# taipingeric/yolo-v4-tf.keras

Measured on AMD Instinct MI355X. Metric: images/sec end-to-end predict() at 608x608 batch 32; conv MFMA %peak, higher is better.
Workload: dtype bf16

## Files before the change

### yolo-v4-tf.keras_amd/csrc/conv_igemm.hip

```cpp
#include "conv_chain.h"
#include "conv_tiles.h"

namespace y4 {

int conv_launch_f32(int tile, const ConvK& k, hipStream_t s);
int conv_launch_bf16(int tile, const ConvK& k, hipStream_t s);
int conv_launch_f16(int tile, const ConvK& k, hipStream_t s);
int conv_launch_bf16_fused(int tile, const ConvK& k, hipStream_t s);
int conv_launch_f16_fused(int tile, const ConvK& k, hipStream_t s);

template <class F, class... A>
static int launch_16bit(int dtype, const char* who, F* bf16, F* f16, const A&... a) {
    if (dtype == Y4_BF16) return bf16(a...);
    if (dtype == Y4_F16) return f16(a...);
    set_error("conv2d: %s 16-bit only", who);
    return Y4_EINVAL;
}
int conv_p8_launch_bf16(int bm, int nst, const ConvK& k, hipStream_t s);
int conv_p8_launch_f16(int bm, int nst, const ConvK& k, hipStream_t s);
int conv_halo_launch_bf16(int bm, int bn, const ConvK& k, hipStream_t s);
int conv_halo_launch_f16(int bm, int bn, const ConvK& k, hipStream_t s);
int conv_halo2_launch_bf16(int tile, const ConvK& k, hipStream_t s);
int conv_halo2_launch_f16(int tile, const ConvK& k, hipStream_t s);
int conv_p8_launch(int dtype, int bm, int nst, const ConvK& k, hipStream_t s) {
    return launch_16bit(dtype, "the phased kernel is", conv_p8_launch_bf16, conv_p8_launch_f16, bm, nst, k, s);
}
int conv_halo_launch(int dtype, int bm, int bn, const ConvK& k, hipStream_t s) {
    return launch_16bit(dtype, "halo tiles are", conv_halo_launch_bf16, conv_halo_launch_f16, bm, bn, k, s);
}
int conv_halo2_launch(int dtype, int tile, const ConvK& k, hipStream_t s) {
    return launch_16bit(dtype, "halo2 tiles are", conv_halo2_launch_bf16, conv_halo2_launch_f16, tile, k, s);
}

int conv_tile_count() { return kNumTiles; }

bool weight_touch_enabled() {
    static const bool on = [] { const char* e = getenv("Y4_NO_WEIGHT_TOUCH"); return !(e && e[0] == '1'); }();
    return on;
}

static bool tile_ok(const TileCfg& tc, int dtype, int cin, int cout_pad) {
    const int bk = tc.bkb / elem_size(dtype);
    return cin % bk == 0 && cout_pad % tc.bn == 0;
}

static void set_bands(ConvK& k, const HaloPlan& hp, int n) {
    k.h_rows = hp.rows; k.h_bands = hp.bands; k.h_pitch = hp.pitch;
    k.h_div_pitch = fastdiv_make((uint32_t)hp.pitch); k.h_div_bands = fastdiv_make((uint32_t)hp.bands);
    k.grid_m = n * hp.bands;
}

int conv_pick_tile(int dtype, int M, int cin, int cout) {
    const int es = elem_size(dtype);
    const bool k128 = cin % (128 / es) == 0;
    if (cout <= 32) return k128 ? 5 : 6;
    if (cout <= 64) return k128 ? 3 : 4;
    return k128 ? 8 : 9;
}

int conv2d_launch(const y4_conv_desc* d, const char* zero_page, hipStream_t stream, const ConvChainDesc* chain,
                  const ConvPairDesc* pair, const ConvObjDesc* obj) {
    Y4_REQUIRE(d && d->in && d->wt && d->out && d->scale && d->shift, Y4_EINVAL, "conv2d: null pointer");
    Y4_REQUIRE(d->dtype >= Y4_F32 && d->dtype <= Y4_F16, Y4_EINVAL, "conv2d: bad dtype %d", d->dtype);
    Y4_REQUIRE(d->ksize == 1 || d->ksize == 3, Y4_EINVAL, "conv2d: ksize %d (only 1 or 3)", d->ksize);
    Y4_REQUIRE(d->stride == 1 || (d->stride == 2 && d->ksize == 3), Y4_EINVAL, "conv2d: stride %d", d->stride);
    Y4_REQUIRE(d->stride == 1 || (d->h % 2 == 0 && d->w % 2 == 0), Y4_EINVAL, "conv2d: stride 2 needs even h,w");
    Y4_REQUIRE(d->n > 0 && d->h > 0 && d->w > 0 && d->cin > 0 && d->cout > 0, Y4_EINVAL, "conv2d: empty shape");
    const int es = elem_size(d->dtype);
    const int epc = 16 / es;
    Y4_REQUIRE(d->cin % (64 / es) == 0, Y4_EINVAL, "conv2d: cin %d must be a multiple of %d for dtype %d",
               d->cin, 64 / es, d->dtype);
    Y4_REQUIRE(d->cin % k_chunk_channels(d->cin, d->ksize) == 0, Y4_EINVAL,
               "conv2d: cin %d is not a whole number of %d-channel K chunks (the canonical K order of a 3x3 conv, common.h)", d->cin,
               k_chunk_channels(d->cin, d->ksize));
    Y4_REQUIRE(d->in_cstride % epc == 0 && d->in_coff % epc == 0, Y4_EINVAL, "conv2d: input view not 16-byte aligned");
    const int oepc = d->out_f32 ? 4 : epc;
    Y4_REQUIRE(d->out_cstride % oepc == 0 && d->out_coff % oepc == 0, Y4_EINVAL,
               "conv2d: output view not 16-byte aligned");
    Y4_REQUIRE(!d->res || (d->res_cstride % epc == 0 && d->res_coff % epc == 0), Y4_EINVAL,
               "conv2d: residual view not 16-byte aligned");
    ConvK k{};
    k.in = (const char*)d->in; k.wt = (const char*)d->wt; k.scale = d->scale; k.shift = d->shift;
    k.res = (const char*)d->res; k.out = (char*)d->out; k.zero = zero_page;
    k.N = d->n; k.H = d->h; k.W = d->w; k.Cin = d->cin;
    k.Ho = d->h / d->stride; k.Wo = d->w / d->stride;
    k.cout_store = (int)round_up(d->cout, 8);
    Y4_REQUIRE((int64_t)d->n * k.Ho * k.Wo < (1ll << 31), Y4_EINVAL, "conv2d: too many output pixels");
    k.M = d->n * k.Ho * k.Wo;
    k.K = d->ksize * d->ksize * d->cin;
    const int64_t in_bytes = (int64_t)d->n * d->h * d->w * d->in_cstride * es;
    const int64_t wt_bytes = (int64_t)round_up(d->cout, COUT_PAD) * k.K * es;
    const int64_t tap_span = d->ksize == 3 ? ((int64_t)3 * d->w + 3) * d->in_cstride * es + (int64_t)d->cin * es : 0;
    Y4_REQUIRE(in_bytes + tap_span < (1ll << 31) && wt_bytes < (1ll << 31), Y4_EINVAL,
               "conv2d: input (%lld B + %lld B of tap reach) or weights (%lld B) exceed the 2 GiB buffer-descriptor range", (long long)in_bytes,
               (long long)tap_span, (long long)wt_bytes);
    k.in_bytes = (unsigned)in_bytes; k.wt_bytes = (unsigned)wt_bytes;
    {
        const int64_t ob = (int64_t)k.M * d->out_cstride * es, ob2 = d->out2 ? (int64_t)k.M * d->out2_cstride * es : 0,
                      rb = d->res ? (int64_t)k.M * d->res_cstride * es : 0;
        k.fast_epi = !d->upsample && !d->out_f32 && ob < (1ll << 31) && ob2 < (1ll << 31) && rb < (1ll << 31);
        if (k.fast_epi) { k.out_bytes = (unsigned)ob; k.out2_bytes = (unsigned)ob2; k.res_bytes = (unsigned)rb; }
    }
    k.div_howo = fastdiv_make((uint32_t)(k.Ho * k.Wo)); k.div_wo = fastdiv_make((uint32_t)k.Wo);
    k.in_cstride = d->in_cstride; k.in_coff = d->in_coff;
    k.out_cstride = d->out_cstride; k.out_coff = d->out_coff;
    k.res_cstride = d->res_cstride; k.res_coff = d->res_coff;
    k.ksize = d->ksize; k.stride = d->stride; k.pad = d->ksize == 3 ? 1 : 0;
    k.act = d->act; k.upsample = d->upsample; k.out_f32 = d->out_f32;
    if (obj) {
        Y4_REQUIRE(obj->obj && !d->upsample && ((pair && pair->out_f32) || (!pair && d->out_f32)), Y4_EINVAL,
                   "conv2d: an objectness side array needs a float32 head");
        k.obj = obj->obj; k.obj_nf = obj->nf; k.obj_cpi = obj->cells_per_img; k.obj_base = obj->cell_base;
    }
    const int cout_pad = (int)round_up(d->cout, COUT_PAD);
    if (pair) {
        Y4_REQUIRE(!chain && d->dtype != Y4_F32 && (d->cout == 128 || d->cout == 256) && pair->cout >= 1 && pair->cout <= d->cout && !d->upsample &&
                       !d->out_f32 && (!d->out2 || (d->split == 64 && d->cout == 128)) && pair->w && pair->scale && pair->shift && pair->fin &&
                       pair->fin_cstride % (pair->out_f32 ? 4 : epc) == 0 && pair->fin_coff % (pair->out_f32 ? 4 : epc) == 0,
                   Y4_EINVAL, "conv2d: bad LDS-pair description");
        k.pair = pair->out_f32 ? 3 : 1; k.tail_act = pair->act; k.store_x = pair->store_x;
        k.tail[0].w = (const char*)pair->w; k.tail[0].scale = pair->scale; k.tail[0].shift = pair->shift; k.tail[0].cout = (int)round_up(pair->cout, 8);
// ... 211 lines not shown
```

### yolo-v4-tf.keras_amd/csrc/conv_igemm_kernel.h

```cpp
#pragma once
#include "conv_chain.h"
#include "conv_tiles.h"

namespace y4 {

#ifdef Y4_TRACE
__device__ unsigned long long y4_trace_buf[4 * 8 * 8];
__device__ unsigned long long y4_trace_life[8 * 8];
#define TR_LIFE(P, INSN)                                                                                    \
    do {                                                                                                    \
        __builtin_amdgcn_sched_barrier(0);                                                                  \
        if (tr_life_on) asm volatile(INSN " %0" : "=s"(tr_life[P]));                                        \
        __builtin_amdgcn_sched_barrier(0);                                                                  \
    } while (0)
#define TR_KT0 10
#define TR_WG 8
#define TR_POINT(P)                                                                                         \
    do {                                                                                                    \
        __builtin_amdgcn_sched_barrier(0);                                                                  \
        if (tr_on && kt >= TR_KT0 && kt < TR_KT0 + 4) asm volatile("s_memtime %0" : "=s"(tr_t[P]));         \
        __builtin_amdgcn_sched_barrier(0);                                                                  \
    } while (0)
#else
#define TR_POINT(P)
#define TR_LIFE(P, INSN)
#endif

template <int DT, int BM, int BN, int WM, int WN, int BKB, int NST, int CHAIN = 0, bool PAIR = false>
__global__ __launch_bounds__(64 * WM * WN, CHAIN ? 2 : 1) void conv_igemm_kernel(const ConvK p) {
    constexpr int NT = 64 * WM * WN;
    constexpr int ES = (DT == Y4_F32) ? 4 : 2;
    constexpr int BK = BKB / ES;
    constexpr int CPR = BKB / 16;
    constexpr int EPC = 16 / ES;
    constexpr int RPI = NT / CPR;
    constexpr int A_IT = (BM + RPI - 1) / RPI;
    constexpr bool A_PART = BM % RPI != 0;
    constexpr int B_IT = BN >= RPI ? BN / RPI : 1;
    constexpr bool B_PART = BN < RPI;
    constexpr int WPX = BM / WM, WCH = BN / WN;
    constexpr int MREP = WPX / 16, NREP = WCH / 16;
    constexpr int CPL = 4 * NREP;
    constexpr bool PHASED = (NST == 12);
    constexpr bool M32 = (NST == 32);
    constexpr int SN = (PHASED || M32) ? 2 : NST;
    constexpr bool PREFRAG = true;
    constexpr int STAGE = (BM + BN) * BKB;
    constexpr int KSTEPS = BKB / 64;
    static_assert(BM % 16 == 0 && (BN % RPI == 0 || (RPI % BN == 0 && (BN * CPR) % 64 == 0)), "tile rows vs rows-per-iteration");
    constexpr int LDS_MAIN = SN * STAGE + (CHAIN ? ChainShape<CHAIN ? CHAIN : 1>::LDS_BYTES : 0);
    static_assert(MREP >= 1 && NREP >= 1, "wave tile");
    constexpr int LPT = A_IT + B_IT;
    static_assert(SN >= 2 && SN <= 7 && (SN == 2 || !B_PART), "deep pipelines need uniform weight loads per wave");
    static_assert((SN - 2) * LPT <= 63, "vmcnt field");
    static_assert(!PHASED || (NT == 512 && KSTEPS == 2), "phased schedule: 8 waves, 128-byte K rows");
    static_assert(!M32 || (DT != Y4_F32 && BKB == 128 && WPX % 32 == 0 && WCH % 32 == 0 && CHAIN == 0 && !PAIR && !B_PART),
                  "32x32x16 tiles: 16-bit, 128-byte K rows, wave tile in 32x32 blocks, plain launches");

    extern __shared__ __attribute__((aligned(16))) char smem[];

    asm volatile("" ::"s"(p.H), "s"(p.W), "s"(p.Cin), "s"(p.Ho), "s"(p.Wo), "s"(p.M), "s"(p.K), "s"(p.in_cstride), "s"(p.in_coff), "s"(p.ksize),
                 "s"(p.stride), "s"(p.pad), "s"(p.grid_m), "s"(p.grid_n), "s"(p.in_bytes), "s"(p.wt_bytes), "s"(p.ksplit), "s"(p.touch));

    const int nwg = p.grid_m * p.grid_n;
    int t, ks = 0;
    {
        const int b = blockIdx.x, qq = nwg >> 3, rr = nwg & 7, xcd = b & 7;
        int idx = b >> 3;
        if constexpr (CHAIN == 0 && !PAIR && NST != 12 && NST != 32) {
            if (p.ksplit > 1) {
                ks = idx % p.ksplit;
                idx /= p.ksplit;
                if (idx >= qq + (xcd < rr ? 1 : 0)) return;
            }
        }
        t = (xcd < rr ? xcd * (qq + 1) : rr * (qq + 1) + (xcd - rr) * qq) + idx;
    }
    const int tile_m = (int)fastdiv((uint32_t)t, p.div_gridn), tile_n = t - tile_m * p.grid_n;
    const int m0 = tile_m * BM, n0 = tile_n * BN;

    const int tid = threadIdx.x, lane = tid & 63, wave = tid >> 6;
    const int wm = wave / WN, wn = wave - wm * WN;
#ifdef Y4_TRACE
#ifndef Y4_TRACE_PAIR
#define Y4_TRACE_PAIR 0
#endif
    const bool tr_life_on = blockIdx.x == TR_WG && BM == Y4_TRACE_BM && BN == 256 && NST == Y4_TRACE_NST && CHAIN == 0 && PAIR == (Y4_TRACE_PAIR != 0);
    unsigned long long tr_life[8] = {0, 0, 0, 0, 0, 0, 0, 0};
#endif
    TR_LIFE(0, "s_memtime");
    TR_LIFE(5, "s_memrealtime");
    ChainPrefetch<CHAIN != 0 ? MREP : 1> chain_pf;
    if constexpr (CHAIN != 0) {
        chain_stage_weights<CHAIN, WM * WN>(p, smem + SN * STAGE, __builtin_amdgcn_readfirstlane(wave), lane);
        chain_prefetch<DT, MREP, CHAIN>(p, chain_pf, m0 + wm * WPX + (lane & 15), p.M, lane);
    }

    const int q = tid % CPR, r0 = tid / CPR;
    auto tswz = [](int row) { return M32 ? (swz<CPR>(row) ^ ((row >> 4) & 1)) : swz<CPR>(row); };
    int a_off[A_IT], a_mask[A_IT];
    const int HoWo = p.Ho * p.Wo;
#pragma unroll
    for (int j = 0; j < A_IT; ++j) {
        const int row = r0 + j * RPI;
        const int m = m0 + row;
        const int mm = m < p.M ? m : 0;
        const int n = (int)fastdiv((uint32_t)mm, p.div_howo), rem = mm - n * HoWo;
        const int ho = (int)fastdiv((uint32_t)rem, p.div_wo), wo = rem - ho * p.Wo;
        const int hi0 = ho * p.stride - p.pad, wi0 = wo * p.stride - p.pad;
        a_off[j] = (((n * p.H + hi0 + 1) * p.W + wi0 + 1) * p.in_cstride + p.in_coff + ((q ^ tswz(row)) * EPC)) * ES;
        int mask = 1;
        if (p.ksize == 3) {
            const int cols = ((unsigned)wi0 < (unsigned)p.W ? 1 : 0) | ((unsigned)(wi0 + 1) < (unsigned)p.W ? 2 : 0) | ((unsigned)(wi0 + 2) < (unsigned)p.W ? 4 : 0);
            mask = ((unsigned)hi0 < (unsigned)p.H ? cols : 0) | ((unsigned)(hi0 + 1) < (unsigned)p.H ? cols << 3 : 0) |
                   ((unsigned)(hi0 + 2) < (unsigned)p.H ? cols << 6 : 0);
        }
        a_mask[j] = m < p.M ? mask : 0;
    }
    int b_off[B_IT];
#pragma unroll
    for (int j = 0; j < B_IT; ++j) {
        const int row = B_PART ? (r0 % BN) : (r0 + j * RPI);
        const int wb = row / WCH, pr = row - wb * WCH;
        int ch;
        if constexpr (M32) {
            const int jb = pr >> 5, R = pr & 31, g = R >> 3, hh = (R >> 2) & 1, jj = R & 3;
            ch = chunk_channel_g<2>(n0 + wb * WCH, 2 * jb + (g >> 1), hh) + (g & 1) * 4 + jj;
        } else {
            const int jn = pr >> 4, i = pr & 15, g = i >> 2, r = i & 3;
            ch = chunk_channel(n0 + wb * WCH, jn >> 1, g) + (jn & 1) * 4 + r;
        }
        b_off[j] = (ch * p.K + ((q ^ tswz(row)) * EPC)) * ES;
    }
    const int tap_bias = (p.W + 1) * p.in_cstride * ES;
    const __amdgpu_buffer_rsrc_t rs_in = make_rsrc(p.in - tap_bias, p.in_bytes + (unsigned)tap_bias);
    const __amdgpu_buffer_rsrc_t rs_wt = make_rsrc(p.wt, p.wt_bytes);
    const int wave_lds = __builtin_amdgcn_readfirstlane(wave * 1024);

    const bool a_skip = A_PART && __builtin_amdgcn_readfirstlane(r0 + (A_IT - 1) * RPI >= BM ? 1 : 0) != 0;
    const int chb = k_chunk_channels(p.Cin, p.ksize) * ES;
    int ky = 0, kx = 0, cbase = 0, c_in = 0, ktb = 0;
    int nk = p.K / BK;
    if constexpr (CHAIN == 0 && !PAIR && NST != 12 && NST != 32) {
        if (p.ksplit > 1) {
            const int kt0 = (int)((int64_t)ks * nk / p.ksplit), kt1 = (int)((int64_t)(ks + 1) * nk / p.ksplit);
            const int per = chb / BKB;
            const int idx = kt0 / per, taps = p.ksize * p.ksize;
            const int chunk = idx / taps, tap = idx - chunk * taps;
            ky = tap / p.ksize; kx = tap - ky * p.ksize;
            cbase = chunk * chb;
            c_in = (kt0 - idx * per) * BKB;
            ktb = kt0 * BKB;
            nk = kt1 - kt0;
        }
    }
    constexpr bool TAPVEC = A_IT <= 2 && SN >= 5;
    typedef int i32x16 __attribute__((ext_vector_type(16)));
    const int cs = p.in_cstride * ES;
    const int step_row = (p.W - (p.ksize - 1)) * cs, step_back = -((p.ksize - 1) * p.W + (p.ksize - 1)) * cs;
    int tap = ky * p.ksize + kx;
    int tap_off = (ky * p.W + kx) * cs;
    int a_vo[A_IT];
    i32x16 a_tapv[TAPVEC ? A_IT : 1];
    if constexpr (TAPVEC) {
#pragma unroll
        for (int j = 0; j < A_IT; ++j)
#pragma unroll
            for (int t = 0; t < 9; ++t) a_tapv[j][t] = ((a_mask[j] >> t) & 1) ? a_off[j] : (int)0x80000000;
    }
    auto set_tap = [&]() {
#pragma unroll
        for (int j = 0; j < A_IT; ++j) {
            if constexpr (TAPVEC) a_vo[j] = a_tapv[j][tap];
            else a_vo[j] = ((a_mask[j] >> tap) & 1) ? a_off[j] : (int)0x80000000;
        }
    };
    set_tap();
    int c0b = cbase + c_in + tap_off;
    auto stage = [&](int buf) {
        const int da = buf * STAGE + wave_lds;
        const int db = da + BM * BKB;
#pragma unroll
        for (int j = 0; j < A_IT; ++j)
            if (!A_PART || r0 + j * RPI < BM)
                buffer_load16_lds(rs_in, smem + da + j * (NT * 16), a_vo[j], c0b);
#pragma unroll
        for (int j = 0; j < B_IT; ++j)
            if (!B_PART || tid < BN * CPR)
                buffer_load16_lds(rs_wt, smem + db + j * (NT * 16), b_off[j], ktb);
        ktb += BKB;
        c_in += BKB;
        if (__builtin_expect(c_in >= chb, 1)) {
            c_in = 0;
            ++tap;
            tap_off += cs;
            if (__builtin_expect(++kx >= p.ksize, 0)) {
                kx = 0;
                tap_off += step_row - cs;
                if (++ky >= p.ksize) { ky = 0; tap = 0; tap_off = 0; cbase += chb; }
            }
            set_tap();
        }
        c0b = cbase + c_in + tap_off;
    };

    if (p.touch != 0) {
        weight_touch(rs_wt, smem + LDS_MAIN, n0 * p.K * ES, BN * p.K * ES, wave, NT / 64, lane);
        if constexpr (PAIR)
            weight_touch(make_rsrc(p.tail[0].w, p.tail_w_bytes), smem + LDS_MAIN, 0, (int)p.tail_w_bytes, wave, NT / 64, lane);
    }

    const int frow = lane & 15, fg = lane >> 4;
    int xo[KSTEPS];
#pragma unroll
    for (int kk = 0; kk < KSTEPS; ++kk) xo[kk] = frow * BKB + (((kk * 4 + fg) ^ swz<CPR>(frow)) * 16);
    const char* const lds_x = smem + (wm * WPX) * BKB;
    const char* const lds_w = smem + BM * BKB + (wn * WCH) * BKB;

    f32x4 acc[MREP][NREP];
#pragma unroll
    for (int i = 0; i < MREP; ++i)
#pragma unroll
        for (int j = 0; j < NREP; ++j) acc[i][j] = f32x4{0.f, 0.f, 0.f, 0.f};

    constexpr bool EARLY_TABLES = CHAIN == 0 && !PAIR && !M32 && !PHASED && NREP <= 2;
    float sc_early[NREP * 4], sh_early[NREP * 4];
    if constexpr (EARLY_TABLES) conv_epilogue_tables<NREP>(p, n0 + wn * WCH, fg, sc_early, sh_early);

    TR_LIFE(1, "s_memtime");
    if constexpr (M32) {
        constexpr int MB = WPX / 32, NB = WCH / 32;
        const int frow32 = lane & 31, fh = lane >> 5;
        int xo32[4];
#pragma unroll
        for (int ks = 0; ks < 4; ++ks) xo32[ks] = frow32 * 128 + (((2 * ks + fh) ^ tswz(frow32)) * 16);
        f32x16 acc32[MB][NB];
#pragma unroll
        for (int i = 0; i < MB; ++i)
#pragma unroll
            for (int j = 0; j < NB; ++j)
#pragma unroll
                for (int e = 0; e < 16; ++e) acc32[i][j][e] = 0.f;
        stage(0);
        for (int kt = 0; kt < nk; ++kt) {
            wait_vmcnt_then_barrier<0>();
            if (kt + 1 < nk) stage((kt + 1) & 1);
            unsigned xa[4], wa[4];
#pragma unroll
            for (int ks = 0; ks < 4; ++ks) {
                xa[ks] = (unsigned)(uintptr_t)(smem + (kt & 1) * STAGE + (wm * WPX) * BKB + xo32[ks]);
                wa[ks] = (unsigned)(uintptr_t)(smem + (kt & 1) * STAGE + (wn * WCH) * BKB + xo32[ks]);
            }
            u32x4 xf[4][MB], wf[4][NB];
#pragma unroll
            for (int ks = 0; ks < 4; ++ks) {
#pragma unroll
                for (int i = 0; i < MB; ++i)
                    asm volatile("ds_read_b128 %0, %1 offset:%2" : "=v"(xf[ks][i]) : "v"(xa[ks]), "n"(i * 32 * 128));
#pragma unroll
                for (int j = 0; j < NB; ++j)
                    asm volatile("ds_read_b128 %0, %1 offset:%2" : "=v"(wf[ks][j]) : "v"(wa[ks]), "n"(BM * BKB + j * 32 * 128));
            }
            __builtin_amdgcn_s_setprio(1);
#pragma unroll
            for (int ks = 0; ks < 4; ++ks) {
                constexpr int R = MB + NB;
                if (ks == 0) asm volatile("s_waitcnt lgkmcnt(%2)" : "+v"(xf[0][0]), "+v"(wf[0][0]) : "n"(3 * R > 15 ? 15 : 3 * R));
                if (ks == 1) asm volatile("s_waitcnt lgkmcnt(%2)" : "+v"(xf[1][0]), "+v"(wf[1][0]) : "n"(2 * R > 15 ? 15 : 2 * R));
                if (ks == 2) asm volatile("s_waitcnt lgkmcnt(%2)" : "+v"(xf[2][0]), "+v"(wf[2][0]) : "n"(R > 15 ? 15 : R));
                if (ks == 3) asm volatile("s_waitcnt lgkmcnt(%2)" : "+v"(xf[3][0]), "+v"(wf[3][0]) : "n"(0));
#pragma unroll
                for (int j = 0; j < NB; ++j)
#pragma unroll
                    for (int i = 0; i < MB; ++i) Mma32<DT>::run(acc32[i][j], wf[ks][j], xf[ks][i]);
                __builtin_amdgcn_sched_barrier(0);
            }
            __builtin_amdgcn_s_setprio(0);
        }
        f32x4 accv[MB][NB * 4];
#pragma unroll
        for (int i = 0; i < MB; ++i)
#pragma unroll
            for (int j = 0; j < NB; ++j)
#pragma unroll
                for (int f = 0; f < 4; ++f)
                    accv[i][j * 4 + f] = f32x4{acc32[i][j][4 * f], acc32[i][j][4 * f + 1], acc32[i][j][4 * f + 2], acc32[i][j][4 * f + 3]};
        const bool full32 = (m0 + BM <= p.M) && (n0 + BN <= p.cout_store);
        conv_epilogue<DT, MB, NB * 4, false, 2>(p, accv, m0 + wm * WPX + frow32, p.M, n0 + wn * WCH, fh, full32);
        return;
    } else if constexpr (PHASED) {
        auto phase_barrier = [] {
            asm volatile("s_barrier" ::: "memory");
            __builtin_amdgcn_sched_barrier(0);
        };
        auto wait_loads = [] { asm volatile("s_waitcnt vmcnt(0)" ::: "memory"); };
        const bool grp1 = __builtin_amdgcn_readfirstlane(wave >= 4 ? 1 : 0) != 0;
        stage(0);
        wait_loads();
        phase_barrier();
        if (grp1) {
            if (nk > 1) stage(1);
            phase_barrier();
        }
        for (int kt = 0; kt < nk; ++kt) {
            const char* sx = lds_x + (kt & 1) * STAGE;
            const char* sw = lds_w + (kt & 1) * STAGE;
            u32x4 xf[MREP], wf[NREP];
            if (!grp1 && kt + 1 < nk) stage((kt + 1) & 1);
#pragma unroll
            for (int i = 0; i < MREP; ++i) xf[i] = *(const u32x4*)(sx + i * 16 * BKB + xo[0]);
#pragma unroll
            for (int j = 0; j < NREP; ++j) wf[j] = *(const u32x4*)(sw + j * 16 * BKB + xo[0]);
            phase_barrier();
// ... 22 lines not shown
        }
        if (!grp1) phase_barrier();
    } else {
#pragma unroll
    for (int s = 0; s < SN - 1; ++s)
        if (s < nk) stage(s);
    int cur = 0, nxt = SN - 1;
#ifdef Y4_TRACE
    const bool tr_on = blockIdx.x == TR_WG && BM == Y4_TRACE_BM && BN == 256 && NST == Y4_TRACE_NST && CHAIN == 0 && !PAIR;
    unsigned long long tr_t[8] = {0, 0, 0, 0, 0, 0, 0, 0};
#endif
    for (int kt = 0; kt < nk; ++kt) {
        TR_POINT(0);
#ifdef Y4_TRACE
        if (tr_on && kt >= TR_KT0 && kt < TR_KT0 + 4) asm volatile("s_memrealtime %0" : "=s"(tr_t[7]));
#endif
        const int ahead = nk - 1 - kt;
#ifdef Y4_TRACE
        if (SN == 2 || ahead == 0) {
            asm volatile("s_waitcnt vmcnt(0)" ::: "memory");
            TR_POINT(4);
            asm volatile("s_barrier" ::: "memory");
        } else
#endif
        if (a_skip) wait_vmcnt_then_barrier_k<SN - 2, LPT - 1>(ahead);
        else wait_vmcnt_then_barrier_k<SN - 2, LPT>(ahead);
        TR_POINT(1);
        if (kt == 0) TR_LIFE(2, "s_memtime");
        constexpr bool READS_FIRST = SN >= 5;
        if (!READS_FIRST && kt + SN - 1 < nk) stage(nxt);
        TR_POINT(2);
        const char* sx = lds_x + cur * STAGE;
        const char* sw = lds_w + cur * STAGE;
        const int nxt_now = nxt;
        cur = cur + 1 == SN ? 0 : cur + 1;
        nxt = nxt + 1 == SN ? 0 : nxt + 1;
        if constexpr (PREFRAG) {
            u32x4 xf[KSTEPS][MREP], wf[KSTEPS][NREP];
#pragma unroll
            for (int kk = 0; kk < KSTEPS; ++kk) {
#pragma unroll
                for (int i = 0; i < MREP; ++i) xf[kk][i] = *(const u32x4*)(sx + i * 16 * BKB + xo[kk]);
#pragma unroll
                for (int j = 0; j < NREP; ++j) wf[kk][j] = *(const u32x4*)(sw + j * 16 * BKB + xo[kk]);
            }
            TR_POINT(3);
            if (READS_FIRST && kt + SN - 1 < nk) stage(nxt_now);
            __builtin_amdgcn_s_setprio(1);
#pragma unroll
            for (int kk = 0; kk < KSTEPS; ++kk)
#pragma unroll
                for (int i = 0; i < MREP; ++i)
#pragma unroll
                    for (int j = 0; j < NREP; ++j) Mma<DT>::run(acc[i][j], wf[kk][j], xf[kk][i]);
            __builtin_amdgcn_s_setprio(0);
            TR_POINT(5);
#ifdef Y4_TRACE
            if (tr_on && kt >= TR_KT0 && kt < TR_KT0 + 4) {
                asm volatile("s_waitcnt lgkmcnt(0)" ::: "memory");
                if (lane == 0)
                    for (int q2 = 0; q2 < 8; ++q2) y4_trace_buf[((kt - TR_KT0) * 8 + wave) * 8 + q2] = tr_t[q2];
            }
#endif
        } else
#pragma unroll
        for (int kk = 0; kk < KSTEPS; ++kk) {
            u32x4 xf[MREP], wf[NREP];
#pragma unroll
            for (int i = 0; i < MREP; ++i) xf[i] = *(const u32x4*)(sx + i * 16 * BKB + xo[kk]);
#pragma unroll
            for (int j = 0; j < NREP; ++j) wf[j] = *(const u32x4*)(sw + j * 16 * BKB + xo[kk]);
#pragma unroll
            for (int i = 0; i < MREP; ++i)
#pragma unroll
                for (int j = 0; j < NREP; ++j) Mma<DT>::run(acc[i][j], wf[j], xf[i]);
        }
    }
    }

    if constexpr (CHAIN != 0) {
        static_assert(WN == 1 && BN == 16 * ChainShape<CHAIN>::HEAD_NREP && DT != Y4_F32,
                      "chain head: one wave column over all its output channels, 16-bit");
        chain_epilogue<DT, MREP, CHAIN>(p, smem + SN * STAGE, acc, chain_pf, m0 + wm * WPX + frow, p.M, lane);
    } else if constexpr (PAIR) {
        static_assert(BKB == 128 && DT != Y4_F32 && SN == 2 && !PHASED && !B_PART, "LDS pair: plain 2-stage, 128-byte rows");
        constexpr int XPANEL = BM * 128, NK2 = BN / 64, XBYTES = NK2 * XPANEL, W2STAGE = BN * 128;
        TR_LIFE(3, "s_memtime");
        __syncthreads();
        char* const xl = smem;
        const int xrow = wm * WPX + frow, mrow = m0 + xrow, chw = wn * WCH;
        int b2_off[B_IT];
#pragma unroll
        for (int j = 0; j < B_IT; ++j) {
            const int row = r0 + j * RPI;
            const int wb = row / WCH, pr = row - wb * WCH;
            const int jn = pr >> 4, i = pr & 15, g = i >> 2, r = i & 3;
            const int ch = chunk_channel(wb * WCH, jn >> 1, g) + (jn & 1) * 4 + r;
            b2_off[j] = (ch * p.tail_k + ((q ^ swz<CPR>(row)) * EPC)) * ES;
        }
        const __amdgpu_buffer_rsrc_t rs_w2 = make_rsrc(p.tail[0].w, p.tail_w_bytes);
        auto stage_w2 = [&](int buf, int kt) {
#pragma unroll
            for (int j = 0; j < B_IT; ++j)
                buffer_load16_lds(rs_w2, smem + XBYTES + buf * W2STAGE + wave_lds + j * (NT * 16), b2_off[j], kt * BKB);
        };
        stage_w2(0, 0);
        conv_epilogue<DT, MREP, NREP, true>(p, acc, mrow, p.M, chw, fg, m0 + BM <= p.M, xl, xrow, XPANEL);
        __syncthreads();
        TR_LIFE(7, "s_memtime");
        f32x4 acc2[MREP][NREP];
#pragma unroll
        for (int i = 0; i < MREP; ++i)
#pragma unroll
            for (int j = 0; j < NREP; ++j) acc2[i][j] = f32x4{0.f, 0.f, 0.f, 0.f};
        const int nk2 = p.tail_k >> 6;
        for (int kt = 0; kt < nk2; ++kt) {
            wait_vmcnt_then_barrier<0>();
            if (kt + 1 < nk2) stage_w2((kt + 1) & 1, kt + 1);
            const char* sx = xl + (p.tail_panel0 + kt) * XPANEL + (wm * WPX) * BKB;
            const char* sw = smem + XBYTES + (kt & 1) * W2STAGE + (wn * WCH) * BKB;
            u32x4 xf[KSTEPS][MREP], wf[KSTEPS][NREP];
#pragma unroll
            for (int kk = 0; kk < KSTEPS; ++kk) {
#pragma unroll
                for (int i = 0; i < MREP; ++i) xf[kk][i] = *(const u32x4*)(sx + i * 16 * BKB + xo[kk]);
#pragma unroll
                for (int j = 0; j < NREP; ++j) wf[kk][j] = *(const u32x4*)(sw + j * 16 * BKB + xo[kk]);
            }
#pragma unroll
            for (int kk = 0; kk < KSTEPS; ++kk)
#pragma unroll
                for (int i = 0; i < MREP; ++i)
#pragma unroll
                    for (int j = 0; j < NREP; ++j) Mma<DT>::run(acc2[i][j], wf[kk][j], xf[kk][i]);
        }
#if defined(Y4_TRACE) && Y4_TRACE_PAIR
        TR_LIFE(0, "s_memtime");
#endif
        ConvK p2 = p;
        p2.scale = p.tail[0].scale; p2.shift = p.tail[0].shift; p2.act = p.tail_act; p2.res = nullptr;
        p2.out = p.fin; p2.out_cstride = p.fin_cstride; p2.out_coff = p.fin_coff;
        p2.cout_store = p.tail[0].cout; p2.upsample = 0; p2.out_f32 = p.pair >> 1;
        p2.split = p.tail_split; p2.out2 = p.fin2; p2.out2_cstride = p.fin2_cstride; p2.out2_coff = p.fin2_coff;
        p2.fast_epi = p.fast_tail; p2.out_bytes = p.fin_bytes; p2.out2_bytes = p.fin2_bytes;
        conv_epilogue<DT, MREP, NREP>(p2, acc2, mrow, p.M, chw, fg, (m0 + BM <= p.M) && BN <= p2.cout_store);
#if defined(Y4_TRACE) && Y4_TRACE_PAIR
        TR_LIFE(1, "s_memtime");
#endif
        if (p.store_x) pair_store_tile<DT, MREP, NREP>(p, xl, xrow, XPANEL, mrow, p.M, chw, fg);
        TR_LIFE(4, "s_memtime");
        TR_LIFE(6, "s_memrealtime");
#ifdef Y4_TRACE
        if (tr_life_on) {
            asm volatile("s_waitcnt lgkmcnt(0)" ::: "memory");
            if (lane == 0)
                for (int q2 = 0; q2 < 8; ++q2) y4_trace_life[wave * 8 + q2] = tr_life[q2];
        }
#endif
    } else {
        TR_LIFE(3, "s_memtime");
        if constexpr (NST != 12 && NST != 32) {
            if (p.ksplit > 1) {
                constexpr int FR = MREP * NREP;
                f32x4* const mine = (f32x4*)p.part + ((size_t)ks * nwg + t) * FR * NT + tid;
#pragma unroll
                for (int i = 0; i < MREP; ++i)
#pragma unroll
                    for (int j = 0; j < NREP; ++j) store16_agent(mine + (i * NREP + j) * NT, acc[i][j]);
                asm volatile("s_waitcnt vmcnt(0)" ::: "memory");
                __syncthreads();
                int* const flag = (int*)smem;
                if (tid == 0) {
                    const int old = atomicAdd(p.split_cnt + t, 1);
                    if (old == p.ksplit - 1) p.split_cnt[t] = 0;
                    *flag = old == p.ksplit - 1;
                }
                __syncthreads();
                if (*flag == 0) return;
                const f32x4* src = (const f32x4*)p.part + (size_t)t * FR * NT + tid;
                for (int sp = 0; sp < p.ksplit; ++sp) {
#pragma unroll
                    for (int i = 0; i < MREP; ++i) {
                        f32x4 part[NREP];
#pragma unroll
                        for (int j = 0; j < NREP; ++j) part[j] = load16_agent(src + (i * NREP + j) * NT);
#pragma unroll
                        for (int j = 0; j < NREP; ++j) acc[i][j] = sp == 0 ? part[j] : acc[i][j] + part[j];
                    }
                    src += (size_t)nwg * FR * NT;
                }
            }
        }
        const bool full = (m0 + BM <= p.M) && (n0 + BN <= p.cout_store);
        if constexpr (EARLY_TABLES) conv_epilogue_with<DT, MREP, NREP>(p, acc, sc_early, sh_early, m0 + wm * WPX + frow, p.M, n0 + wn * WCH, fg, full);
        else conv_epilogue<DT, MREP, NREP>(p, acc, m0 + wm * WPX + frow, p.M, n0 + wn * WCH, fg, full);
        TR_LIFE(4, "s_memtime");
        TR_LIFE(6, "s_memrealtime");
#ifdef Y4_TRACE
        if (tr_life_on) {
            asm volatile("s_waitcnt lgkmcnt(0)" ::: "memory");
            if (lane == 0)
                for (int q2 = 0; q2 < 8; ++q2) y4_trace_life[wave * 8 + q2] = tr_life[q2];
        }
#endif
    }
}

template <int DT, int BM, int BN, int WM, int WN, int BKB, int NST, int CHAIN = 0, bool PAIR = false>
static int launch_cfg(const ConvK& k, hipStream_t stream) {
    constexpr int lds_main = (NST == 12 || NST == 32 ? 2 : NST) * (BM + BN) * BKB + (CHAIN ? ChainShape<CHAIN ? CHAIN : 1>::LDS_BYTES : 0) + TOUCH_LDS;
    constexpr int lds_pair = PAIR ? (BN / 64) * BM * 128 + 2 * BN * 128 : 0;
    constexpr int lds = lds_main > lds_pair ? lds_main : lds_pair;
    static_assert(lds <= 160 * 1024, "LDS budget");
    constexpr int lds_limit = lds > 48 * 1024 ? lds : 0;
    int grid = k.grid_m * k.grid_n;
    if (k.ksplit > 1) {
        Y4_REQUIRE(CHAIN == 0 && !PAIR && NST != 12 && NST != 32, Y4_EINVAL, "conv2d: this tile / fusion cannot run split-K");
        const int nwg = k.grid_m * k.grid_n, per_xcd = (nwg >> 3) + ((nwg & 7) ? 1 : 0);
        grid = 8 * per_xcd * k.ksplit;
    }
    return launch_lds<conv_igemm_kernel<DT, BM, BN, WM, WN, BKB, NST, CHAIN, PAIR>>(lds_limit, dim3(grid), dim3(64 * WM * WN), lds, stream, k);
}

int conv_p8_launch(int dtype, int bm, int nst, const ConvK& k, hipStream_t s);
int conv_halo_launch(int dtype, int bm, int bn, const ConvK& k, hipStream_t s);
int conv_halo2_launch(int dtype, int tile, const ConvK& k, hipStream_t s);

template <int DT>
static int launch_plain(int tile, const ConvK& k, hipStream_t s) {
#define Y4_TILE_CASE(id, bm, bn, wm, wn, bkb, nst)                                            \
    case id:                                                                                  \
        if constexpr (DT == Y4_F32 && !f32_tile(id)) break;                                   \
        else if constexpr (DT == Y4_F32 && nst == 32) break;                                  \
        else if constexpr (nst == 8 || nst == 9 || nst == 10) return conv_p8_launch(DT, bm, nst, k, s); \
        else if constexpr (nst == 20) return conv_halo_launch(DT, bm, bn, k, s);              \
        else if constexpr (nst == 21) return conv_halo2_launch(DT, id, k, s);                 \
        else return launch_cfg<DT, bm, bn, wm, wn, bkb, nst>(k, s);
    switch (tile) { Y4_TILES(Y4_TILE_CASE) }
    set_error("conv2d: tile id %d is not available for this dtype", tile);
    return Y4_EINVAL;
}

template <int DT>
static int launch_fused(int tile, const ConvK& k, hipStream_t s) {
    if (k.pair) {
        if constexpr (DT != Y4_F32) {
#define Y4_PAIR_CASE(id, bm, bn, wm, wn) case id: return launch_cfg<DT, bm, bn, wm, wn, 128, 2, 0, true>(k, s);
            switch (tile) {
                Y4_PAIR_CASE(1, 128, 128, 2, 2) Y4_PAIR_CASE(8, 64, 128, 1, 4) Y4_PAIR_CASE(20, 96, 128, 2, 2)
                Y4_PAIR_CASE(24, 160, 128, 2, 2) Y4_PAIR_CASE(25, 192, 128, 2, 2) Y4_PAIR_CASE(29, 112, 128, 1, 4)
                Y4_PAIR_CASE(13, 128, 256, 2, 4) Y4_PAIR_CASE(19, 192, 256, 2, 4) Y4_PAIR_CASE(21, 96, 256, 2, 4)
                Y4_PAIR_CASE(22, 160, 256, 2, 4) Y4_PAIR_CASE(38, 384, 128, 4, 2)
                case 51: return conv_halo_launch(DT, 384, 128, k, s);
                case 52: return conv_halo_launch(DT, 192, 256, k, s);
                case 54: return conv_halo_launch(DT, 320, 128, k, s);
            }
#undef Y4_PAIR_CASE
        }
        set_error("conv2d: tile id %d cannot head an LDS pair", tile);
        return Y4_EINVAL;
    }
    if (k.ntail > 0) {
        if constexpr (DT != Y4_F32) {
            const int cfg = k.ntail == 1 ? 1 : (k.tail[0].w == nullptr ? 4 : (k.tail[1].cout == 64 ? 2 : 3));
#define Y4_CHAIN_CASE(CFG)                                                                   \
    case CFG:                                                                                \
        switch (tile) {                                                                      \
            case 3: return launch_cfg<DT, 128, 64, 4, 1, 128, 2, CFG>(k, s);                 \
            case 4: return launch_cfg<DT, 128, 64, 4, 1, 64, 2, CFG>(k, s);                  \
            case 15: return launch_cfg<DT, 128, 64, 4, 1, 64, 4, CFG>(k, s);                 \
        }                                                                                    \
        break;
            switch (cfg) { Y4_CHAIN_CASE(1) Y4_CHAIN_CASE(2) Y4_CHAIN_CASE(3) Y4_CHAIN_CASE(4) }
#undef Y4_CHAIN_CASE
        }
        set_error("conv2d: tile id %d cannot head a chain", tile);
        return Y4_EINVAL;
    }
    set_error("conv2d: not a fused launch");
    return Y4_EINVAL;
}

}
```

Measured before the change: 6509.

## Make fused pair conv kernel persistent and prefetch next tile under tail

The fused pair kernel (a conv whose output stays in LDS and feeds a second 1x1 tail conv) becomes persistent. The grid is capped at the number of resident slots (CUs times occupancy, overridable by an environment variable), and each workgroup walks a strided run of tiles within its XCD. Where no intermediate store is needed, the next tile's first input stages are issued before the tail epilogue so the global loads overlap it. Launch bounds allow two blocks per CU for small 4-wave pair tiles. This removes launch and tail-wave imbalance and hides prologue latency, at the cost of more register pressure and more complex indexing, including an m0 recompute that assumes grid_n is 1.

```diff
diff --git a/yolo-v4-tf.keras_amd/csrc/conv_igemm.hip b/yolo-v4-tf.keras_amd/csrc/conv_igemm.hip
--- a/yolo-v4-tf.keras_amd/csrc/conv_igemm.hip
+++ b/yolo-v4-tf.keras_amd/csrc/conv_igemm.hip
@@ -37,6 +37,11 @@
 bool weight_touch_enabled() {
     static const bool on = [] { const char* e = getenv("Y4_NO_WEIGHT_TOUCH"); return !(e && e[0] == '1'); }();
     return on;
+}
+
+int pair_slots_cap() {
+    static const int cap = [] { const char* e = getenv("Y4_PAIR_SLOTS"); const int v = e ? atoi(e) : 0; return v > 0 ? v : 0; }();
+    return cap;
 }
 
 static bool tile_ok(const TileCfg& tc, int dtype, int cin, int cout_pad) {
diff --git a/yolo-v4-tf.keras_amd/csrc/conv_igemm_kernel.h b/yolo-v4-tf.keras_amd/csrc/conv_igemm_kernel.h
--- a/yolo-v4-tf.keras_amd/csrc/conv_igemm_kernel.h
+++ b/yolo-v4-tf.keras_amd/csrc/conv_igemm_kernel.h
@@ -27,7 +27,7 @@
 #endif
 
 template <int DT, int BM, int BN, int WM, int WN, int BKB, int NST, int CHAIN = 0, bool PAIR = false>
-__global__ __launch_bounds__(64 * WM * WN, CHAIN ? 2 : 1) void conv_igemm_kernel(const ConvK p) {
+__global__ __launch_bounds__(64 * WM * WN, (CHAIN || (PAIR && WM * WN == 4 && BM <= 128)) ? 2 : 1) void conv_igemm_kernel(const ConvK p) {
     constexpr int NT = 64 * WM * WN;
     constexpr int ES = (DT == Y4_F32) ? 4 : 2;
     constexpr int BK = BKB / ES;
@@ -64,7 +64,15 @@
 
     const int nwg = p.grid_m * p.grid_n;
     int t, ks = 0;
-    {
+    [[maybe_unused]] int t_end = 0, t_step = 0;
+    if constexpr (PAIR) {
+        const int G = gridDim.x, b = blockIdx.x, nx = G >= 8 ? 8 : G, xcd = G >= 8 ? (b & 7) : b;
+        t_step = G >= 8 ? ((G - xcd + 7) >> 3) : 1;
+        const int qq = G >= 8 ? (nwg >> 3) : nwg / nx, rr = nwg - qq * nx;
+        t = (xcd < rr ? xcd * (qq + 1) : rr * (qq + 1) + (xcd - rr) * qq) + (G >= 8 ? (b >> 3) : 0);
+        t_end = t - (G >= 8 ? (b >> 3) : 0) + qq + (xcd < rr ? 1 : 0);
+        if (t >= t_end) return;
+    } else {
         const int b = blockIdx.x, qq = nwg >> 3, rr = nwg & 7, xcd = b & 7;
         int idx = b >> 3;
         if constexpr (CHAIN == 0 && !PAIR && NST != 12 && NST != 32) {
@@ -77,7 +85,8 @@
         t = (xcd < rr ? xcd * (qq + 1) : rr * (qq + 1) + (xcd - rr) * qq) + idx;
     }
     const int tile_m = (int)fastdiv((uint32_t)t, p.div_gridn), tile_n = t - tile_m * p.grid_n;
-    const int m0 = tile_m * BM, n0 = tile_n * BN;
+    int m0 = tile_m * BM;
+    const int n0 = tile_n * BN;
 
     const int tid = threadIdx.x, lane = tid & 63, wave = tid >> 6;
     const int wm = wave / WN, wn = wave - wm * WN;
@@ -100,23 +109,25 @@
     auto tswz = [](int row) { return M32 ? (swz<CPR>(row) ^ ((row >> 4) & 1)) : swz<CPR>(row); };
     int a_off[A_IT], a_mask[A_IT];
     const int HoWo = p.Ho * p.Wo;
-#pragma unroll
-    for (int j = 0; j < A_IT; ++j) {
-        const int row = r0 + j * RPI;
-        const int m = m0 + row;
-        const int mm = m < p.M ? m : 0;
-        const int n = (int)fastdiv((uint32_t)mm, p.div_howo), rem = mm - n * HoWo;
-        const int ho = (int)fastdiv((uint32_t)rem, p.div_wo), wo = rem - ho * p.Wo;
-        const int hi0 = ho * p.stride - p.pad, wi0 = wo * p.stride - p.pad;
-        a_off[j] = (((n * p.H + hi0 + 1) * p.W + wi0 + 1) * p.in_cstride + p.in_coff + ((q ^ tswz(row)) * EPC)) * ES;
-        int mask = 1;
-        if (p.ksize == 3) {
-            const int cols = ((unsigned)wi0 < (unsigned)p.W ? 1 : 0) | ((unsigned)(wi0 + 1) < (unsigned)p.W ? 2 : 0) | ((unsigned)(wi0 + 2) < (unsigned)p.W ? 4 : 0);
-            mask = ((unsigned)hi0 < (unsigned)p.H ? cols : 0) | ((unsigned)(hi0 + 1) < (unsigned)p.H ? cols << 3 : 0) |
-                   ((unsigned)(hi0 + 2) < (unsigned)p.H ? cols << 6 : 0);
-        }
-        a_mask[j] = m < p.M ? mask : 0;
-    }
+#define Y4_TILE_ROWS(M_FIRST)                                                                                                            \
+    _Pragma("unroll") for (int j = 0; j < A_IT; ++j) {                                                                                   \
+        const int row = r0 + j * RPI;                                                                                                    \
+        const int m = (M_FIRST) + row;                                                                                                   \
+        const int mm = m < p.M ? m : 0;                                                                                                  \
+        const int n = (int)fastdiv((uint32_t)mm, p.div_howo), rem = mm - n * HoWo;                                                       \
+        const int ho = (int)fastdiv((uint32_t)rem, p.div_wo), wo = rem - ho * p.Wo;                                                      \
+        const int hi0 = ho * p.stride - p.pad, wi0 = wo * p.stride - p.pad;                                                              \
+        a_off[j] = (((n * p.H + hi0 + 1) * p.W + wi0 + 1) * p.in_cstride + p.in_coff + ((q ^ tswz(row)) * EPC)) * ES;                    \
+        int mask = 1;                                                                                                                    \
+        if (p.ksize == 3) {                                                                                                              \
+            const int cols = ((unsigned)wi0 < (unsigned)p.W ? 1 : 0) | ((unsigned)(wi0 + 1) < (unsigned)p.W ? 2 : 0) |                   \
+                             ((unsigned)(wi0 + 2) < (unsigned)p.W ? 4 : 0);                                                              \
+            mask = ((unsigned)hi0 < (unsigned)p.H ? cols : 0) | ((unsigned)(hi0 + 1) < (unsigned)p.H ? cols << 3 : 0) |                  \
+                   ((unsigned)(hi0 + 2) < (unsigned)p.H ? cols << 6 : 0);                                                                \
+        }                                                                                                                                \
+        a_mask[j] = m < p.M ? mask : 0;                                                                                                  \
+    }
+    Y4_TILE_ROWS(m0)
     int b_off[B_IT];
 #pragma unroll
     for (int j = 0; j < B_IT; ++j) {
@@ -228,7 +239,149 @@
     if constexpr (EARLY_TABLES) conv_epilogue_tables<NREP>(p, n0 + wn * WCH, fg, sc_early, sh_early);
 
     TR_LIFE(1, "s_memtime");
-    if constexpr (M32) {
+    if constexpr (PAIR) {
+        static_assert(BKB == 128 && DT != Y4_F32 && SN == 2 && !PHASED && !M32 && !B_PART && CHAIN == 0, "LDS pair: plain 2-stage, 128-byte rows");
+        constexpr int XPANEL = BM * 128, NK2 = BN / 64, XBYTES = NK2 * XPANEL, W2STAGE = BN * 128;
+        static_assert(SN * STAGE <= XBYTES + 2 * W2STAGE, "the K loop's stages lie inside the panels + the tail's weight stages");
+        constexpr bool UNDER_TAIL = NT == 512;
+        char* const xl = smem;
+        const int xrow_wg = wm * WPX + frow, chw_wg = wn * WCH, fg_wg = fg;
+        int b2_off[B_IT];
+#pragma unroll
+        for (int j = 0; j < B_IT; ++j) {
+            const int row = r0 + j * RPI;
+            const int wb = row / WCH, pr = row - wb * WCH;
+            const int jn = pr >> 4, i = pr & 15, g = i >> 2, r = i & 3;
+            const int ch = chunk_channel(wb * WCH, jn >> 1, g) + (jn & 1) * 4 + r;
+            b2_off[j] = (ch * p.tail_k + ((q ^ swz<CPR>(row)) * EPC)) * ES;
+        }
+        const __amdgpu_buffer_rsrc_t rs_w2 = make_rsrc(p.tail[0].w, p.tail_w_bytes);
+        auto stage_w2 = [&](int buf, int kt) {
+#pragma unroll
+            for (int j = 0; j < B_IT; ++j)
+                buffer_load16_lds(rs_w2, smem + XBYTES + buf * W2STAGE + wave_lds + j * (NT * 16), b2_off[j], kt * BKB);
+        };
+        auto per_tile = [](const float* tab) {
+            asm volatile("" : "+s"(tab));
+            return tab;
+        };
+        const int nk2 = p.tail_k >> 6;
+        auto stage_first_two = [&]() {
+            stage(0);
+            if (nk > 1) stage(1);
+        };
+        auto reads_done_then_barrier = [] { asm volatile("s_waitcnt lgkmcnt(0)\n\ts_barrier" ::: "memory"); };
+        stage_first_two();
+#ifdef Y4_TRACE
+        int tr_tiles = 0;
+#endif
+        for (;;) {
+            int xrow = xrow_wg, chw = chw_wg, fg = fg_wg;
+            asm volatile("" : "+v"(xrow), "+v"(chw), "+v"(fg));
+            const int mrow = m0 + xrow;
+#pragma unroll
+            for (int i = 0; i < MREP; ++i)
+#pragma unroll
+                for (int j = 0; j < NREP; ++j) acc[i][j] = f32x4{0.f, 0.f, 0.f, 0.f};
+            for (int kt = 0; kt < nk; ++kt) {
+                wait_vmcnt_then_barrier<0>();
+                if (kt == 0) TR_LIFE(2, "s_memtime");
+                if (kt > 0 && kt + 1 < nk) stage((kt + 1) & 1);
+                const char* sx = lds_x + (kt & 1) * STAGE;
+                const char* sw = lds_w + (kt & 1) * STAGE;
+                u32x4 xf[KSTEPS][MREP], wf[KSTEPS][NREP];
+#pragma unroll
+                for (int kk = 0; kk < KSTEPS; ++kk) {
+#pragma unroll
+                    for (int i = 0; i < MREP; ++i) xf[kk][i] = *(const u32x4*)(sx + i * 16 * BKB + xo[kk]);
+#pragma unroll
+                    for (int j = 0; j < NREP; ++j) wf[kk][j] = *(const u32x4*)(sw + j * 16 * BKB + xo[kk]);
+                }
+                __builtin_amdgcn_s_setprio(1);
+#pragma unroll
+                for (int kk = 0; kk < KSTEPS; ++kk)
+#pragma unroll
+                    for (int i = 0; i < MREP; ++i)
+#pragma unroll
+                        for (int j = 0; j < NREP; ++j) Mma<DT>::run(acc[i][j], wf[kk][j], xf[kk][i]);
+                __builtin_amdgcn_s_setprio(0);
+            }
+            TR_LIFE(3, "s_memtime");
+            __syncthreads();
+            stage_w2(0, 0);
+            ConvK p1 = p;
+            p1.scale = per_tile(p.scale); p1.shift = per_tile(p.shift);
+            conv_epilogue<DT, MREP, NREP, true>(p1, acc, mrow, p.M, chw, fg, m0 + BM <= p.M, xl, xrow, XPANEL);
+            __syncthreads();
+            TR_LIFE(7, "s_memtime");
+            f32x4 acc2[MREP][NREP];
+#pragma unroll
+            for (int i = 0; i < MREP; ++i)
+#pragma unroll
+                for (int j = 0; j < NREP; ++j) acc2[i][j] = f32x4{0.f, 0.f, 0.f, 0.f};
+            for (int kt = 0; kt < nk2; ++kt) {
+                wait_vmcnt_then_barrier<0>();
+                if (kt + 1 < nk2) stage_w2((kt + 1) & 1, kt + 1);
+                const char* sx = xl + (p.tail_panel0 + kt) * XPANEL + (wm * WPX) * BKB;
+                const char* sw = smem + XBYTES + (kt & 1) * W2STAGE + (wn * WCH) * BKB;
+                u32x4 xf[KSTEPS][MREP], wf[KSTEPS][NREP];
+#pragma unroll
+                for (int kk = 0; kk < KSTEPS; ++kk) {
+#pragma unroll
+                    for (int i = 0; i < MREP; ++i) xf[kk][i] = *(const u32x4*)(sx + i * 16 * BKB + xo[kk]);
+#pragma unroll
+                    for (int j = 0; j < NREP; ++j) wf[kk][j] = *(const u32x4*)(sw + j * 16 * BKB + xo[kk]);
+                }
+#pragma unroll
+                for (int kk = 0; kk < KSTEPS; ++kk)
+#pragma unroll
+                    for (int i = 0; i < MREP; ++i)
+#pragma unroll
+                        for (int j = 0; j < NREP; ++j) Mma<DT>::run(acc2[i][j], wf[kk][j], xf[kk][i]);
+            }
+#if defined(Y4_TRACE) && Y4_TRACE_PAIR
+            TR_LIFE(0, "s_memtime");
+#endif
+            const int m_this = m0;
+            const bool more = t + t_step < t_end;
+            auto next_tile = [&]() {
+                t += t_step;
+                m0 = t * BM;
+                Y4_TILE_ROWS(m0)
+                cbase = 0; ktb = 0; c0b = 0;
+                set_tap();
+                reads_done_then_barrier();
+                stage_first_two();
+            };
+            bool early = false;
+            if constexpr (UNDER_TAIL) early = !p.store_x;
+            if (more && early) next_tile();
+            ConvK p2 = p;
+            p2.scale = per_tile(p.tail[0].scale); p2.shift = per_tile(p.tail[0].shift); p2.act = p.tail_act; p2.res = nullptr;
+            p2.out = p.fin; p2.out_cstride = p.fin_cstride; p2.out_coff = p.fin_coff;
+            p2.cout_store = p.tail[0].cout; p2.upsample = 0; p2.out_f32 = p.pair >> 1;
+            p2.split = p.tail_split; p2.out2 = p.fin2; p2.out2_cstride = p.fin2_cstride; p2.out2_coff = p.fin2_coff;
+            p2.fast_epi = p.fast_tail; p2.out_bytes = p.fin_bytes; p2.out2_bytes = p.fin2_bytes;
+            conv_epilogue<DT, MREP, NREP>(p2, acc2, mrow, p.M, chw, fg, (m_this + BM <= p.M) && BN <= p2.cout_store);
+#if defined(Y4_TRACE) && Y4_TRACE_PAIR
+            TR_LIFE(1, "s_memtime");
+#endif
+            if (p.store_x) pair_store_tile<DT, MREP, NREP>(p, xl, xrow, XPANEL, mrow, p.M, chw, fg);
+            if (more && !early) next_tile();
+            TR_LIFE(4, "s_memtime");
+            TR_LIFE(6, "s_memrealtime");
+#ifdef Y4_TRACE
+            if (tr_life_on && tr_tiles < 2) {
+                asm volatile("s_waitcnt lgkmcnt(0)" ::: "memory");
+                if (lane == 0)
+                    for (int q2 = 0; q2 < 8; ++q2) y4_trace_life[wave * 8 + q2] = tr_life[q2];
+            }
+            ++tr_tiles;
+            TR_LIFE(5, "s_memrealtime");
+#endif
+            if (!more) return;
+        }
+    } else if constexpr (M32) {
         constexpr int MB = WPX / 32, NB = WCH / 32;
         const int frow32 = lane & 31, fh = lane >> 5;
         int xo32[4];
@@ -417,81 +570,6 @@
         static_assert(WN == 1 && BN == 16 * ChainShape<CHAIN>::HEAD_NREP && DT != Y4_F32,
                       "chain head: one wave column over all its output channels, 16-bit");
         chain_epilogue<DT, MREP, CHAIN>(p, smem + SN * STAGE, acc, chain_pf, m0 + wm * WPX + frow, p.M, lane);
-    } else if constexpr (PAIR) {
-        static_assert(BKB == 128 && DT != Y4_F32 && SN == 2 && !PHASED && !B_PART, "LDS pair: plain 2-stage, 128-byte rows");
-        constexpr int XPANEL = BM * 128, NK2 = BN / 64, XBYTES = NK2 * XPANEL, W2STAGE = BN * 128;
-        TR_LIFE(3, "s_memtime");
-        __syncthreads();
-        char* const xl = smem;
-        const int xrow = wm * WPX + frow, mrow = m0 + xrow, chw = wn * WCH;
-        int b2_off[B_IT];
-#pragma unroll
-        for (int j = 0; j < B_IT; ++j) {
-            const int row = r0 + j * RPI;
-            const int wb = row / WCH, pr = row - wb * WCH;
-            const int jn = pr >> 4, i = pr & 15, g = i >> 2, r = i & 3;
-            const int ch = chunk_channel(wb * WCH, jn >> 1, g) + (jn & 1) * 4 + r;
-            b2_off[j] = (ch * p.tail_k + ((q ^ swz<CPR>(row)) * EPC)) * ES;
-        }
-        const __amdgpu_buffer_rsrc_t rs_w2 = make_rsrc(p.tail[0].w, p.tail_w_bytes);
-        auto stage_w2 = [&](int buf, int kt) {
-#pragma unroll
-            for (int j = 0; j < B_IT; ++j)
-                buffer_load16_lds(rs_w2, smem + XBYTES + buf * W2STAGE + wave_lds + j * (NT * 16), b2_off[j], kt * BKB);
-        };
-        stage_w2(0, 0);
-        conv_epilogue<DT, MREP, NREP, true>(p, acc, mrow, p.M, chw, fg, m0 + BM <= p.M, xl, xrow, XPANEL);
-        __syncthreads();
-        TR_LIFE(7, "s_memtime");
-        f32x4 acc2[MREP][NREP];
-#pragma unroll
-        for (int i = 0; i < MREP; ++i)
-#pragma unroll
-            for (int j = 0; j < NREP; ++j) acc2[i][j] = f32x4{0.f, 0.f, 0.f, 0.f};
-        const int nk2 = p.tail_k >> 6;
-        for (int kt = 0; kt < nk2; ++kt) {
-            wait_vmcnt_then_barrier<0>();
-            if (kt + 1 < nk2) stage_w2((kt + 1) & 1, kt + 1);
-            const char* sx = xl + (p.tail_panel0 + kt) * XPANEL + (wm * WPX) * BKB;
-            const char* sw = smem + XBYTES + (kt & 1) * W2STAGE + (wn * WCH) * BKB;
-            u32x4 xf[KSTEPS][MREP], wf[KSTEPS][NREP];
-#pragma unroll
-            for (int kk = 0; kk < KSTEPS; ++kk) {
-#pragma unroll
-                for (int i = 0; i < MREP; ++i) xf[kk][i] = *(const u32x4*)(sx + i * 16 * BKB + xo[kk]);
-#pragma unroll
-                for (int j = 0; j < NREP; ++j) wf[kk][j] = *(const u32x4*)(sw + j * 16 * BKB + xo[kk]);
-            }
-#pragma unroll
-            for (int kk = 0; kk < KSTEPS; ++kk)
-#pragma unroll
-                for (int i = 0; i < MREP; ++i)
-#pragma unroll
-                    for (int j = 0; j < NREP; ++j) Mma<DT>::run(acc2[i][j], wf[kk][j], xf[kk][i]);
-        }
-#if defined(Y4_TRACE) && Y4_TRACE_PAIR
-        TR_LIFE(0, "s_memtime");
-#endif
-        ConvK p2 = p;
-        p2.scale = p.tail[0].scale; p2.shift = p.tail[0].shift; p2.act = p.tail_act; p2.res = nullptr;
-        p2.out = p.fin; p2.out_cstride = p.fin_cstride; p2.out_coff = p.fin_coff;
-        p2.cout_store = p.tail[0].cout; p2.upsample = 0; p2.out_f32 = p.pair >> 1;
-        p2.split = p.tail_split; p2.out2 = p.fin2; p2.out2_cstride = p.fin2_cstride; p2.out2_coff = p.fin2_coff;
-        p2.fast_epi = p.fast_tail; p2.out_bytes = p.fin_bytes; p2.out2_bytes = p.fin2_bytes;
-        conv_epilogue<DT, MREP, NREP>(p2, acc2, mrow, p.M, chw, fg, (m0 + BM <= p.M) && BN <= p2.cout_store);
-#if defined(Y4_TRACE) && Y4_TRACE_PAIR
-        TR_LIFE(1, "s_memtime");
-#endif
-        if (p.store_x) pair_store_tile<DT, MREP, NREP>(p, xl, xrow, XPANEL, mrow, p.M, chw, fg);
-        TR_LIFE(4, "s_memtime");
-        TR_LIFE(6, "s_memrealtime");
-#ifdef Y4_TRACE
-        if (tr_life_on) {
-            asm volatile("s_waitcnt lgkmcnt(0)" ::: "memory");
-            if (lane == 0)
-                for (int q2 = 0; q2 < 8; ++q2) y4_trace_life[wave * 8 + q2] = tr_life[q2];
-        }
-#endif
     } else {
         TR_LIFE(3, "s_memtime");
         if constexpr (NST != 12 && NST != 32) {
@@ -541,6 +619,10 @@
     }
 }
 
+#undef Y4_TILE_ROWS
+
+int pair_slots_cap();
+
 template <int DT, int BM, int BN, int WM, int WN, int BKB, int NST, int CHAIN = 0, bool PAIR = false>
 static int launch_cfg(const ConvK& k, hipStream_t stream) {
     constexpr int lds_main = (NST == 12 || NST == 32 ? 2 : NST) * (BM + BN) * BKB + (CHAIN ? ChainShape<CHAIN ? CHAIN : 1>::LDS_BYTES : 0) + TOUCH_LDS;
@@ -553,6 +635,23 @@
         Y4_REQUIRE(CHAIN == 0 && !PAIR && NST != 12 && NST != 32, Y4_EINVAL, "conv2d: this tile / fusion cannot run split-K");
         const int nwg = k.grid_m * k.grid_n, per_xcd = (nwg >> 3) + ((nwg & 7) ? 1 : 0);
         grid = 8 * per_xcd * k.ksplit;
+    }
+    if constexpr (PAIR) {
+        static const int per_cu = [] {
+            int nb = 0;
+            if (lds_limit > 0)
+                (void)hipFuncSetAttribute((const void*)conv_igemm_kernel<DT, BM, BN, WM, WN, BKB, NST, CHAIN, PAIR>, hipFuncAttributeMaxDynamicSharedMemorySize, lds_limit);
+            if (hipOccupancyMaxActiveBlocksPerMultiprocessor(&nb, conv_igemm_kernel<DT, BM, BN, WM, WN, BKB, NST, CHAIN, PAIR>, 64 * WM * WN, lds) != hipSuccess || nb < 1) {
+                (void)hipGetLastError();
+                nb = 1;
+            }
+            return nb;
+        }();
+        int cus = 0;
+        if (int r = cu_count(&cus)) return r;
+        int slots = (cus & ~7) * per_cu;
+        if (const int cap = pair_slots_cap()) slots = cap;
+        if (grid > slots) grid = slots > 8 ? (slots & ~7) : slots;
     }
     return launch_lds<conv_igemm_kernel<DT, BM, BN, WM, WN, BKB, NST, CHAIN, PAIR>>(lds_limit, dim3(grid), dim3(64 * WM * WN), lds, stream, k);
 }
```

Result: no change. 6480 (-0.4%).
